# rdesc/autorally

Hardware: AMD Instinct MI355X
Metric: trajectory rollouts/s per MPPI solve (higher is better)
Workload: dtype f32

## Files before the change

autorally_amd/csrc/group_roles.hpp:

```cpp
#pragma once

#include "mppi_device.hpp"
#include "noise_device.hpp"

namespace mppi {

constexpr int kGRing = 16;
constexpr int kGCtlChunk = 4;

template <class SH>
struct GroupRoles {
  static constexpr int kPose = SH::NW, kCost = SH::NW + 1, kCtl = SH::NW + 2, kRng = SH::NW + 3;
  static constexpr int kWaves = SH::NW + 4;
  static_assert(kWaves <= (int)(sizeof(SH::fin) / sizeof(int)), "fin[]");
  static_assert(SH::kR == 16 || SH::kR == 8, "rollouts per group");
};
template <class SH>
__device__ __forceinline__ int group_j(int slot) { return slot & (SH::kR - 1); }
template <class SH>
__device__ __forceinline__ bool group_real(int slot) { return slot < SH::kR; }

template <class SH>
__device__ __forceinline__ int group_seq_min(SH &sh)
{
  int m = lds_peek(lds_addr(&sh.xseq[0][0]));
#pragma unroll
  for (int w = 1; w < SH::NW; w++) m = min(m, lds_peek(lds_addr(&sh.xseq[w][0])));
  return m;
}

struct MrgHalf {
  uint32_t s0, s1, s2;
};
__device__ __forceinline__ uint32_t fold_m(uint64_t x, uint32_t C, uint32_t m)
{
  x = (x >> 32) * C + (x & 0xffffffffULL);
  x = (x >> 32) * C + (x & 0xffffffffULL);
  x = (x >> 32) * C + (x & 0xffffffffULL);
  if (x >= m) x -= m;
  return (uint32_t)x;
}
template <class SH>
__device__ __forceinline__ MrgHalf group_rng_load(const RolloutArgs &a)
{
  const int lane = threadIdx.x & 63;
  const int j = group_j<SH>((lane >> 1) & 15), c = lane & 1;
  const int k = (int)blockIdx.x * SH::kR + j;
  const int K = a.K;
  MrgHalf g{0, 0, 0};
  if (a.inline_noise != 0 && lane < 2 * kRolloutsPerWave) {
    g.s0 = a.rng_in[(3 * c) * K + k]; g.s1 = a.rng_in[(3 * c + 1) * K + k]; g.s2 = a.rng_in[(3 * c + 2) * K + k];
  }
  return g;
}
template <class SH, bool PRE = false>
__device__ __forceinline__ void group_rng_wave(const RolloutArgs &a, SH &sh, const MrgHalf pre = MrgHalf{0, 0, 0})
{
  using R = GroupRoles<SH>;
  const int lane = threadIdx.x & 63;
  const int j = group_j<SH>((lane >> 1) & 15), c = lane & 1;
  const int k = (int)blockIdx.x * SH::kR + j;
  const int K = a.K, T = a.T;
  const bool active = lane < 2 * kRolloutsPerWave;
  const bool real = lane < 2 * SH::kR;
  int budget = spin_budget_init(a.spin_budget, T, a.fault_wave == R::kRng + 1);
  if (a.inline_noise != 0) {
    const uint32_t m = c ? (uint32_t)kM2 : (uint32_t)kM1, C = c ? kC2 : kC1;
    const uint32_t A = c ? (uint32_t)kA21 : (uint32_t)kA12, Bn = c ? (uint32_t)kA23N : (uint32_t)kA13N;
    MrgHalf g{0, 0, 0};
    if constexpr (PRE) {
      g = pre;
    } else if (active) {
      g.s0 = a.rng_in[(3 * c) * K + k]; g.s1 = a.rng_in[(3 * c + 1) * K + k]; g.s2 = a.rng_in[(3 * c + 2) * K + k];
    }
    const uint32_t a_ctl = lds_addr(&sh.ctl_pub[0]);
    const uint32_t a_mypub = lds_addr(&sh.rng_pub[lane]);
    int seen = 0;
    for (int t = 0; t < T; t++) {
      float2 e = make_float2(0.5f, 0.5f);
#ifdef MPPI_DIAG_NORNG
      e = make_float2(0.25f + 0.001f * (float)t, 0.5f);
#else
#pragma unroll
      for (int d = 0; d < 2; d++) {
        const uint32_t p = fold_m((uint64_t)A * (c ? g.s2 : g.s1) + (uint64_t)Bn * (m - g.s0), C, m);
        g.s0 = g.s1; g.s1 = g.s2; g.s2 = p;
        const uint32_t p2 = (uint32_t)__builtin_amdgcn_mov_dpp((int)p, 0xB1, 0xF, 0xF, false);
        uint32_t z = (p >= p2) ? p - p2 : p + (uint32_t)kM1 - p2;
        if (z == 0) z = (uint32_t)kM1;
        const float u = (float)z * 0x1p-32f;
        if (d == 0) e.x = u; else e.y = u;
      }
#endif
      const int need = t - kGRing + 1;
      while (seen < need && --budget > 0) {
        seen = lds_peek(a_ctl);
        if (seen < need) __builtin_amdgcn_s_sleep(2);
      }
      if (active && c == 0) *reinterpret_cast<float2 *>(&sh.eps[t & (kGRing - 1)][j][0]) = e;
      lds_publish(a_mypub, t + 1);
    }
    if (real) {
      a.rng_out[(3 * c) * K + k] = g.s0; a.rng_out[(3 * c + 1) * K + k] = g.s1; a.rng_out[(3 * c + 2) * K + k] = g.s2;
    }
  }
  spin_finish(budget, lds_addr(&sh.fail[0]), lds_addr(&sh.fin[R::kRng]));
}

template <class SH>
__device__ __forceinline__ void group_control_wave(const RolloutArgs &a, SH &sh, const uint32_t a_gate_open = 0)
{
  using R = GroupRoles<SH>;
  constexpr int NSW = SH::NSW;
  static_assert(kGCtlChunk == 4 && kGRing >= 2 * kGCtlChunk, "four steps per iteration, lanes 16 q + j");
  const int lane = threadIdx.x & 63;
  const int j = group_j<SH>(lane & 15), q = lane >> 4;
  const bool real = group_real<SH>(lane & 15);
  const int k = (int)blockIdx.x * SH::kR + j;
  const int K = a.K, T = a.T;
  const bool inl = a.inline_noise != 0;
  float2 *const noise = reinterpret_cast<float2 *>(a.noise);
  const float2 *const Useq = reinterpret_cast<const float2 *>(a.U);
  const bool noise_free_k = (k == 0);
  const bool pure_noise_k = (k >= a.k99);
  const uint32_t a_cd = lds_addr(&sh.cost_done[0]);
  const uint32_t a_mypub = lds_addr(&sh.ctl_pub[lane]);
  const uint32_t a_rng = lds_addr(&sh.rng_pub[0]);
  int budget = spin_budget_init(a.spin_budget, T, a.fault_wave == R::kCtl + 1);
  const bool gated = a_gate_open != 0;
  if (gated)
    while (lds_peek(a_gate_open) == 0 && --budget > 0) __builtin_amdgcn_s_sleep(1);
  int seen_x = 0, seen_c = 0, seen_r = 0;
  for (int t0 = 0, n = 1; t0 < T; t0 += n, n = kGCtlChunk) {
    const int t = t0 + q;
    const bool live = (t < T) & (q < n);
    const int tl = live ? t : T - 1;
    float2 Ut;
    if (gated) {
      const unsigned long long ub = __hip_atomic_load(reinterpret_cast<const unsigned long long *>(Useq + tl), __ATOMIC_RELAXED, __HIP_MEMORY_SCOPE_SYSTEM);
      Ut = make_float2(__uint_as_float((unsigned)ub), __uint_as_float((unsigned)(ub >> 32)));
    } else {
      Ut = Useq[tl];
    }
    float2 e = (live && !inl) ? noise[(size_t)tl * K + k] : make_float2(0.0f, 0.0f);
    const int tm = min(t0 + n, T) - 1;
    const int need_x = (tm >= kGRing) ? (tm - kGRing) * NSW + 1 : 0;
    const int need_c = tm - kGRing + 1;
    while ((seen_x < need_x || seen_c < need_c) && --budget > 0) {
      seen_x = group_seq_min(sh);
      seen_c = lds_peek(a_cd);
      if (seen_x < need_x || seen_c < need_c) __builtin_amdgcn_s_sleep(2);
    }
    if (inl) {
      while (seen_r < tm + 1 && --budget > 0) {
        seen_r = lds_peek(a_rng);
        if (seen_r < tm + 1) __builtin_amdgcn_s_sleep(1);
      }
#ifdef MPPI_DIAG_NOBM
      e = *reinterpret_cast<const float2 *>(&sh.eps[tl & (kGRing - 1)][j][0]);
#else
      e = box_muller(*reinterpret_cast<const float2 *>(&sh.eps[tl & (kGRing - 1)][j][0]));
#endif
    }
    if (live) {
      const bool nf = noise_free_k | (t < a.opt_delay);
      const float n0 = e.x * a.nu[0], n1 = e.y * a.nu[1];
      const float du0 = nf ? 0.0f : n0, du1 = nf ? 0.0f : n1;
      float u0 = nf ? Ut.x : (pure_noise_k ? n0 : Ut.x + n0);
      float u1 = nf ? Ut.y : (pure_noise_k ? n1 : Ut.y + n1);
      if (real) noise[(size_t)t * K + k] = make_float2(u0, u1);
      u0 = clampf(u0, a.u_lo[0], a.u_hi[0]);
      u1 = clampf(u1, a.u_lo[1], a.u_hi[1]);
      const int slot = t & (kGRing - 1);
      sh.ctl_b1[slot][j] = u0;
      sh.ctl_b1[slot][kRolloutsPerWave + j] = u1;
      *reinterpret_cast<float4 *>(&sh.ctl_rec[slot][j][0]) = make_float4(u0, u1, du0, du1);
    }
    lds_publish(a_mypub, tm + 1);
  }
  spin_finish(budget, lds_addr(&sh.fail[0]), lds_addr(&sh.fin[R::kCtl]));
}

template <class SH, bool AFFINE>
__device__ __forceinline__ void group_pose_wave(const RolloutArgs &a, SH &sh)
{
  using R = GroupRoles<SH>;
  constexpr int NSW = SH::NSW;
  static_assert(SH::kR == 16, "one step per iteration: 16-rollout groups only");
  const int lane = threadIdx.x & 63;
  const int j = lane & 15;
  const int T = a.T;
  const uint32_t a_seq0 = lds_addr(&sh.xseq[0][0]);
  const uint32_t a_cd = lds_addr(&sh.cost_done[0]);
  const uint32_t a_mypub = lds_addr(&sh.pose_pub[lane]);
  float x = a.state[0], y = a.state[1], yaw = a.state[2];
  int budget = spin_budget_init(a.spin_budget, T, a.fault_wave == R::kPose + 1), seen = 0, cdone = 0;
  float tf_p = 0.0f, tb_p = 0.0f;
  for (int t = 0; t <= T; t++) {
    float tf = 0.0f, tb = 0.0f;
    if (t < T) {
      const int need = t * NSW + 1;
      while (seen < need && --budget > 0) {
        seen = SH::kRecByAll ? group_seq_min(sh) : lds_peek(a_seq0);
        if (seen < need) __builtin_amdgcn_s_sleep(1);
      }
      const float4 r0 = *reinterpret_cast<const float4 *>(&sh.rec[t & (kGRing - 1)][j][0]);
      float spsi, cpsi;
#ifdef MPPI_DIAG_NOPOSE
      spsi = 0.0f; cpsi = 1.0f; tf = x; tb = y;
#else
      sincos_fast(yaw, spsi, cpsi);
      const float st[3] = {x, y, yaw};
      track_fetch<AFFINE>(a.cost, st, cpsi, spsi, tf, tb);
#endif
      const float sd0 = fmaf(cpsi, r0.y, -(spsi * r0.z));
      const float sd1 = fmaf(spsi, r0.y, cpsi * r0.z);
      const float sd2 = a.negate_yaw_der ? -r0.w : r0.w;
      x = fmaf(sd0, a.dt, x);
      y = fmaf(sd1, a.dt, y);
      yaw = fmaf(sd2, a.dt, yaw);
    }
    if (t > 0) {
      while (cdone < t - kGRing && --budget > 0) cdone = lds_peek(a_cd);
      if (lane < kRolloutsPerWave) *reinterpret_cast<float2 *>(&sh.tex[(t - 1) & (kGRing - 1)][lane][0]) = make_float2(tf_p, tb_p);
      lds_publish(a_mypub, t);
    }
    tf_p = tf; tb_p = tb;
  }
  spin_finish(budget, lds_addr(&sh.fail[0]), lds_addr(&sh.fin[R::kPose]));
}

template <int Q>
__device__ __forceinline__ float quad_bc(float v)
{
  return __int_as_float(__builtin_amdgcn_mov_dpp(__float_as_int(v), Q * 0x55, 0xF, 0xF, false));
}
__device__ __forceinline__ void quad_chain(float v, float d, float dt, int q, float &vq, float &v_out)
{
  const float v1 = fmaf(quad_bc<0>(d), dt, v);
  const float v2 = fmaf(quad_bc<1>(d), dt, v1);
  const float v3 = fmaf(quad_bc<2>(d), dt, v2);
  v_out = fmaf(quad_bc<3>(d), dt, v3);
  const float lo = (q == 0) ? v : v1, hi = (q == 2) ? v2 : v3;
  vq = (q < 2) ? lo : hi;
}
template <class SH, bool AFFINE>
__device__ __forceinline__ void group_pose_wave4(const RolloutArgs &a, SH &sh, const float x0, const float y0, const float yaw0,
                                                 const int budget_cut = 0);
template <class SH, bool AFFINE>
__device__ __forceinline__ void group_pose_wave4(const RolloutArgs &a, SH &sh)
{
  group_pose_wave4<SH, AFFINE>(a, sh, a.state[0], a.state[1], a.state[2]);
}
template <class SH, bool AFFINE>
__device__ __forceinline__ void group_pose_wave4(const RolloutArgs &a, SH &sh, const float x0, const float y0, const float yaw0,
                                                 const int budget_cut)
{
  using R = GroupRoles<SH>;
  constexpr int NSW = SH::NSW;
  static_assert(kRolloutsPerWave == 16 && kGRing >= 8, "lane = 4 j + q");
  const int lane = threadIdx.x & 63;
  const int j = group_j<SH>(lane >> 2), q = lane & 3;
  const int T = a.T;
  const uint32_t a_seq0 = lds_addr(&sh.xseq[0][0]);
  const uint32_t a_cd = lds_addr(&sh.cost_done[0]);
  const uint32_t a_mypub = lds_addr(&sh.pose_pub[lane]);
  float x = x0, y = y0, yaw = yaw0;
  int budget = spin_budget_init(a.spin_budget, T, a.fault_wave == R::kPose + 1 || budget_cut != 0), seen = 0, cdone = 0;
  for (int t0 = 0; t0 < T; t0 += 4) {
    const int t = t0 + q;
    const int tend = min(t0 + 4, T);
    const int need = (tend - 1) * NSW + 1;
    while (seen < need && --budget > 0) {
      seen = SH::kRecByAll ? group_seq_min(sh) : lds_peek(a_seq0);
      if (seen < need) __builtin_amdgcn_s_sleep(1);
    }
    const float4 r0 = *reinterpret_cast<const float4 *>(&sh.rec[t & (kGRing - 1)][j][0]);
    float yaw_q, yaw_n, x_q, x_n, y_q, y_n;
    quad_chain(yaw, a.negate_yaw_der ? -r0.w : r0.w, a.dt, q, yaw_q, yaw_n);
    float spsi, cpsi, tf = 0.0f, tb = 0.0f;
#ifdef MPPI_DIAG_NOPOSE
    spsi = 0.0f; cpsi = 1.0f;
#else
    sincos_fast(yaw_q, spsi, cpsi);
#endif
    quad_chain(x, fmaf(cpsi, r0.y, -(spsi * r0.z)), a.dt, q, x_q, x_n);
    quad_chain(y, fmaf(spsi, r0.y, cpsi * r0.z), a.dt, q, y_q, y_n);
#ifdef MPPI_DIAG_NOPOSE
    tf = x_q; tb = y_q;
#else
    const float st[3] = {x_q, y_q, yaw_q};
    track_fetch<AFFINE>(a.cost, st, cpsi, spsi, tf, tb);
#endif
    x = x_n; y = y_n; yaw = yaw_n;
    while (cdone < tend - kGRing && --budget > 0) cdone = lds_peek(a_cd);
    if (t < T) *reinterpret_cast<float2 *>(&sh.tex[t & (kGRing - 1)][j][0]) = make_float2(tf, tb);
    lds_publish(a_mypub, tend);
  }
  spin_finish(budget, lds_addr(&sh.fail[0]), lds_addr(&sh.fin[R::kPose]));
}

template <class SH>
__device__ __forceinline__ float group_settle(SH &sh, int budget, float J)
{
  using R = GroupRoles<SH>;
  const int lane = threadIdx.x & 63;
  const uint32_t a_fin = lds_addr(&sh.fin[(lane < R::kWaves) ? lane : 0]);
  for (;;) {
    const int v = (lane == R::kCost) ? 1 : lds_peek_lanes(a_fin);
    const bool all = __builtin_amdgcn_ballot_w64(v != 0) == ~0ull;
    if (all || --budget <= 0) break;
    __builtin_amdgcn_s_sleep(1);
  }
  if (budget <= 0 || lds_peek(lds_addr(&sh.fail[0])) != 0) J = __builtin_nanf("");
  return J;
}

template <class SH, bool CTRL>
__device__ __forceinline__ void group_cost_wave(const RolloutArgs &a, SH &sh)
{
  using R = GroupRoles<SH>;
  const int lane = threadIdx.x & 63;
  static_assert(SH::kR == 16, "one step per iteration: 16-rollout groups only");
  const int j = lane & 15;
  const int k = (int)blockIdx.x * kRolloutsPerWave + j;
  const int T = a.T;
  const uint32_t a_mydone = lds_addr(&sh.cost_done[lane]);
  const uint32_t a_pose = lds_addr(&sh.pose_pub[0]);
  int crash = 0, budget = spin_budget_init(a.spin_budget, T, a.fault_wave == R::kCost + 1), seen = 0;
  float J = 0.0f;
  for (int t = 0; t < T; t++) {
    const double rt = a.inv_t[t];
    while (seen < t + 1 && --budget > 0) {
      seen = lds_peek(a_pose);
      if (seen < t + 1) __builtin_amdgcn_s_sleep(1);
    }
    const float4 r0 = *reinterpret_cast<const float4 *>(&sh.rec[t & (kGRing - 1)][j][0]);
    const float4 r1 = *reinterpret_cast<const float4 *>(&sh.ctl_rec[t & (kGRing - 1)][j][0]);
    const float2 tx = *reinterpret_cast<const float2 *>(&sh.tex[t & (kGRing - 1)][j][0]);
    lds_publish(a_mydone, t + 1);
    const int rc = (int)((t > 0) & (fabsf(r0.x) >= kRollCrash));
#ifdef MPPI_DIAG_NOCOST
    crash |= rc;
    int crash_new = crash;
    const float Jn = J + r0.y + r1.x + tx.x + (float)rt;
#else
    CostTerms ct;
    cost_terms_a<CTRL>(a.cost, a.nu, r0.y, r0.z, r1.x, r1.y, r1.z, r1.w, ct);
    crash |= rc;
    int crash_new = crash;
    const float c = cost_terms_b(a.cost, ct, tx.x, tx.y, crash_new);
    const float Jn = running_mean(J, c, t, rt);
#endif
    J = (t > 0) ? Jn : J;
    crash = (t > 0) ? crash_new : crash;
  }
  J = group_settle(sh, budget, J);
  a.costs[k] = J + 0.0f;
}

template <int Q>
__device__ __forceinline__ int quad_bc_i(int v)
{
  return __builtin_amdgcn_mov_dpp(v, Q * 0x55, 0xF, 0xF, false);
}
template <class SH, bool CTRL>
__device__ __forceinline__ void group_cost_wave4(const RolloutArgs &a, SH &sh)
{
  using R = GroupRoles<SH>;
  const int lane = threadIdx.x & 63;
  const int j = group_j<SH>(lane >> 2), q = lane & 3;
  const int k = (int)blockIdx.x * SH::kR + j;
  const int T = a.T;
  const uint32_t a_mydone = lds_addr(&sh.cost_done[lane]);
  const uint32_t a_pose = lds_addr(&sh.pose_pub[0]);
  int crash = 0, budget = spin_budget_init(a.spin_budget, T, a.fault_wave == R::kCost + 1), seen = 0;
  float J = 0.0f;
  for (int t0 = 0; t0 < T; t0 += 4) {
    const int t = t0 + q;
    const int tend = min(t0 + 4, T);
    while (seen < tend && --budget > 0) {
      seen = lds_peek(a_pose);
      if (seen < tend) __builtin_amdgcn_s_sleep(1);
    }
    const float4 r0 = *reinterpret_cast<const float4 *>(&sh.rec[t & (kGRing - 1)][j][0]);
    const float4 r1 = *reinterpret_cast<const float4 *>(&sh.ctl_rec[t & (kGRing - 1)][j][0]);
    const float2 tx = *reinterpret_cast<const float2 *>(&sh.tex[t & (kGRing - 1)][j][0]);
    lds_publish(a_mydone, tend);
    const bool counted = (t > 0) & (t < T);
    int e = (int)(fabsf(r0.x) >= kRollCrash) | (int)(tx.x >= a.cost.boundary_threshold) | (int)(tx.y >= a.cost.boundary_threshold);
    e = counted ? e : 0;
    const int c0 = crash | quad_bc_i<0>(e), c1 = c0 | quad_bc_i<1>(e), c2 = c1 | quad_bc_i<2>(e), c3 = c2 | quad_bc_i<3>(e);
    const int lo = (q == 0) ? c0 : c1, hi = (q == 2) ? c2 : c3;
    int crash_q = (q < 2) ? lo : hi;
    crash = c3;
#ifdef MPPI_DIAG_NOCOST
    const float c = r0.y + r1.x + tx.x + (float)crash_q;
#else
    CostTerms ct;
    cost_terms_a<CTRL>(a.cost, a.nu, r0.y, r0.z, r1.x, r1.y, r1.z, r1.w, ct);
    const float c = cost_terms_b(a.cost, ct, tx.x, tx.y, crash_q);
#endif
#pragma unroll
    for (int l = 0; l < 4; l++) {
      const int tl = t0 + l;
      const float cl = (l == 0) ? quad_bc<0>(c) : (l == 1) ? quad_bc<1>(c) : (l == 2) ? quad_bc<2>(c) : quad_bc<3>(c);
      if (tl > 0 && tl < T) {
#ifdef MPPI_DIAG_NOCOST
        J = J + cl + (float)a.inv_t[tl];
#else
        J = running_mean(J, cl, tl, a.inv_t[tl]);
#endif
      }
    }
  }
  J = group_settle(sh, budget, J);
  if (q == 0 && group_real<SH>(lane >> 2)) a.costs[k] = J + 0.0f;
}

}
```

autorally_amd/csrc/rollout_m44.hip:

```cpp
#include "group_roles.hpp"
#include "mppi_kernels.hpp"

namespace mppi {

typedef float m44_f4 __attribute__((ext_vector_type(4)));
constexpr int kM44H = 64;

struct M44Shared {
  static constexpr int NW = 4;
  static constexpr int NSW = 1;
  static constexpr int kR = 16;
  static constexpr bool kRecByAll = true;
  int xseq[NW][64];
  float rec[kGRing][kRolloutsPerWave][4];
  int cost_done[64];
  float ctl_b1[kGRing][64];
  float ctl_rec[kGRing][kRolloutsPerWave][4];
  int ctl_pub[64];
  float tex[kGRing][kRolloutsPerWave][2];
  int pose_pub[64];
  float eps[kGRing][kRolloutsPerWave][2];
  int rng_pub[64];
  int fail[4];
  int fin[8];
  float gstate[8];
  int gate_open[8];
  m44_f4 wo[4][64];
  float dump[NW][64 * kGRing];
};

template <int NHID>
constexpr int m44_q_bias() { return 2; }
template <int NHID>
constexpr int m44_q_hidden() { return 2 + (NHID + 3) / 4; }
template <int NHID>
constexpr int m44_q_out() { return m44_q_hidden<NHID>() + (NHID - 1) * 16; }
template <int NHID>
constexpr int m44_q_total() { return m44_q_out<NHID>() + 5; }

template <int Q>
__device__ __forceinline__ float m44_qp(float v)
{
  return __int_as_float(__builtin_amdgcn_mov_dpp(__float_as_int(v), Q, 0xF, 0xF, false));
}
__device__ __forceinline__ void m44_transpose(const float (&in)[4], float (&out)[4], bool hi, bool od)
{
  float t[4];
  {
    const float x0 = m44_qp<0x4E>(hi ? in[0] : in[2]);
    const float x1 = m44_qp<0x4E>(hi ? in[1] : in[3]);
    t[0] = hi ? x0 : in[0];
    t[2] = hi ? in[2] : x0;
    t[1] = hi ? x1 : in[1];
    t[3] = hi ? in[3] : x1;
  }
  {
    const float y0 = m44_qp<0xB1>(od ? t[0] : t[1]);
    const float y1 = m44_qp<0xB1>(od ? t[2] : t[3]);
    out[0] = od ? y0 : t[0];
    out[1] = od ? t[1] : y0;
    out[2] = od ? y1 : t[2];
    out[3] = od ? t[3] : y1;
  }
}

template <int K>
__device__ __forceinline__ void m44_step(m44_f4 &d, const float (&T)[4], const float *w)
{
  d = __builtin_amdgcn_mfma_f32_4x4x1f32(T[K & 3], w[K], d, 4, K >> 2, 0);
}
template <int K0>
__device__ __forceinline__ void m44_steps16(m44_f4 &d, const float (&T)[4], const float *w)
{
#define S4(K) m44_step<K>(d, T, w); m44_step<K + 1>(d, T, w); m44_step<K + 2>(d, T, w); m44_step<K + 3>(d, T, w);
  S4(K0) S4(K0 + 4) S4(K0 + 8) S4(K0 + 12)
#undef S4
}
__device__ __forceinline__ void m44_tanh(const m44_f4 &d, float bs, float (&act)[4])
{
  const f32x2 a01 = tanh_bias2(f32x2{d[0], d[1]}, f32x2{bs, bs});
  const f32x2 a23 = tanh_bias2(f32x2{d[2], d[3]}, f32x2{bs, bs});
  act[0] = a01.x; act[1] = a01.y; act[2] = a23.x; act[3] = a23.y;
}

template <int CTRL>
__device__ __forceinline__ float m44_dpp_add(float acc, float src)
{
  return acc + __int_as_float(__builtin_amdgcn_update_dpp(0, __float_as_int(src), CTRL, 0xF, 0xF, true));
}
__device__ __forceinline__ float m44_out_tree(const f32x2 (&q)[4], const f32x2 (&p)[4], const float (&T)[4])
{
  f32x2 Q = q[0] * f32x2{T[0], T[0]}, P = p[0] * f32x2{T[0], T[0]};
#pragma unroll
  for (int s = 1; s < 4; s++) {
    Q = __builtin_elementwise_fma(q[s], f32x2{T[s], T[s]}, Q);
    P = __builtin_elementwise_fma(p[s], f32x2{T[s], T[s]}, P);
  }
  {
    auto x = __builtin_amdgcn_permlane32_swap(__float_as_uint(Q.x), __float_as_uint(P.x), false, false);
// ... 231 lines not shown
```

autorally_amd/csrc/rollout_oct.hip:

```cpp
#include "mfma_net.hpp"
#include "group_roles.hpp"
#include "mppi_kernels.hpp"

namespace mppi {

template <int H, int NHID>
struct OctShared {
  static constexpr int NW = 4;
  static constexpr int NSW = NHID;
  static constexpr int kR = 16;
  static constexpr bool kRecByAll = false;
  float xb[2][NW][64][4];
  int xseq[NW][64];
  float rec[kGRing][kRolloutsPerWave][4];
  int cost_done[64];
  float ctl_b1[kGRing][64];
  float ctl_rec[kGRing][kRolloutsPerWave][4];
  int ctl_pub[64];
  float tex[kGRing][kRolloutsPerWave][2];
  int pose_pub[64];
  float eps[kGRing][kRolloutsPerWave][2];
  int rng_pub[64];
  int fail[4];
  int fin[8];
};

__device__ __forceinline__ void oct_poll(const uint32_t (&a_seq)[3], const uint32_t (&a_x)[3], int &f, f32x4 (&oth)[3])
{
  int f0, f1, f2;
  asm volatile(
      "ds_read_b32 %0, %6\n\tds_read_b128 %3, %9\n\t"
      "ds_read_b32 %1, %7\n\tds_read_b128 %4, %10\n\t"
      "ds_read_b32 %2, %8\n\tds_read_b128 %5, %11\n\t"
      "s_waitcnt lgkmcnt(0)"
      : "=&v"(f0), "=&v"(f1), "=&v"(f2), "=&v"(oth[0]), "=&v"(oth[1]), "=&v"(oth[2])
      : "v"(a_seq[0]), "v"(a_seq[1]), "v"(a_seq[2]), "v"(a_x[0]), "v"(a_x[1]), "v"(a_x[2])
      : "memory");
  f = __builtin_amdgcn_readfirstlane(min(min(f0, f1), f2));
}

template <int H, int NHID, int W>
__device__ __forceinline__ void oct_dynamics(const RolloutArgs &a, OctShared<H, NHID> &sh)
{
  using N = MfmaNet<H, NHID>;
  constexpr int MT = N::MT, KSH = N::KSH, NSW = NHID;
  static_assert(MT == 4, "one M tile per dynamics wave: 64-wide hidden layers");
  const int lane = threadIdx.x & 63;
  const int j = lane & 15, g = lane >> 4;
  const int T = a.T;

  float A0[2], B0[4], AH[(NHID - 1) * KSH + 1], Bh[(NHID - 1) * 4 + 1], AL[KSH], BL[4];
  A0[0] = a.wpack[(W * 2 + 0) * 64 + lane];
  A0[1] = a.wpack[(W * 2 + 1) * 64 + lane];
#pragma unroll
  for (int r = 0; r < 4; r++) B0[r] = a.wpack[(N::nA + W * 4 + r) * 64 + lane] * kTanhScale;
#pragma unroll
  for (int l = 1; l < NHID; l++) {
#pragma unroll
    for (int s = 0; s < KSH; s++)
      AH[(l - 1) * KSH + s] = a.wpack[(N::nA0 + (l - 1) * N::nAH + W * KSH + s) * 64 + lane];
#pragma unroll
    for (int r = 0; r < 4; r++) Bh[(l - 1) * 4 + r] = a.wpack[(N::nA + l * MT * 4 + W * 4 + r) * 64 + lane] * kTanhScale;
  }
#pragma unroll
  for (int s = 0; s < KSH; s++) AL[s] = a.wpack[(N::nA0 + (NHID - 1) * N::nAH + s) * 64 + lane];
#pragma unroll
  for (int r = 0; r < 4; r++) BL[r] = a.wpack[(N::nA + NHID * MT * 4 + r) * 64 + lane];

  const uint32_t a_myseq = lds_addr(&sh.xseq[W][lane]);
  const uint32_t a_xmine = lds_addr(&sh.xb[0][W][lane][0]);
  uint32_t a_seq[3], a_xo[3];
#pragma unroll
  for (int i = 0; i < 3; i++) {
    a_seq[i] = lds_addr(&sh.xseq[(W + 1 + i) & 3][0]);
    a_xo[i] = lds_addr(&sh.xb[0][(W + 1 + i) & 3][lane][0]);
  }
  const uint32_t a_pub = lds_addr(&sh.ctl_pub[0]);
  const uint32_t a_cd = lds_addr(&sh.cost_done[0]);
  constexpr uint32_t kXbParity = 4 * 64 * 4 * 4;

  typedef const volatile int __attribute__((address_space(3))) *lds_int_p;
  typedef const volatile float __attribute__((address_space(3))) *lds_float_p;
  const lds_int_p p_pub = (lds_int_p)&sh.ctl_pub[0];
  const lds_int_p p_cd = (lds_int_p)&sh.cost_done[0];
  const lds_float_p p_b1 = (lds_float_p)&sh.ctl_b1[0][lane];

  float s3 = a.state[3], s4 = a.state[4], s5 = a.state[5], s6 = a.state[6];
  int budget = spin_budget_init(a.spin_budget, T, a.fault_wave == W + 1);
  while (lds_peek(a_pub) < 1 && --budget > 0) __builtin_amdgcn_s_sleep(1);
  float b1_next = sh.ctl_b1[0][lane];
  asm volatile("" : "+v"(b1_next));
  int cp_v = 0, cd_v = 0;
  float b1n_v = 0.0f;

// ... 140 lines not shown
```

autorally_amd/csrc/rollout_row.hip:

```cpp
#include "group_roles.hpp"
#include "mppi_kernels.hpp"

namespace mppi {

#ifdef MPPI_ROW_STAMPS
__device__ unsigned long long g_row_stamps[16];
#define RSTAMP(i)                                                                                         \
  do {                                                                                                    \
    if (blockIdx.x == 0 && (threadIdx.x & 63) == 0) {                                                     \
      unsigned long long t__;                                                                             \
      asm volatile("s_memtime %0\n\ts_waitcnt lgkmcnt(0)" : "=s"(t__)::"memory");                           \
      g_row_stamps[i] = t__;                                                                              \
    }                                                                                                     \
  } while (0)
#else
#define RSTAMP(i) do { } while (0)
#endif

template <int H>
struct RowShared {
  static constexpr int NW = 4;
  static constexpr int NSW = 1;
  static constexpr bool kRecByAll = true;
  static constexpr int kR = 16;
  int xseq[NW][64];
  float rec[kGRing][kRolloutsPerWave][4];
  int cost_done[64];
  float ctl_b1[kGRing][64];
  float ctl_rec[kGRing][kRolloutsPerWave][4];
  int ctl_pub[64];
  float tex[kGRing][kRolloutsPerWave][2];
  int pose_pub[64];
  float eps[kGRing][kRolloutsPerWave][2];
  int rng_pub[64];
  int fail[4];
  int fin[8];
  float gstate[8];
  int gate_open[8];
  float dump[NW][64 * 2 + (kGRing - 1) * kRolloutsPerWave * 4];
};

template <int H, bool TREE>
struct RowWeights {
  f32x2 w1[kNetIn], w2[H], w3[TREE ? 4 : H];
  f32x2 b1s, b2s, b3;
};

constexpr int kRowPackEntries = 40;
template <int H, bool TREE>
__device__ __forceinline__ void row_load(const float *rowpack, int p, RowWeights<H, TREE> &W)
{
  static_assert(H == 32, "entry layout of pack_row_weights");
  const float4 *pk = reinterpret_cast<const float4 *>(rowpack) + p;
#pragma unroll
  for (int i = 0; i < 3; i++) {
    const float4 v = pk[i * 16];
    W.w1[2 * i] = f32x2{v.x, v.y};
    W.w1[2 * i + 1] = f32x2{v.z, v.w};
  }
#pragma unroll
  for (int i = 0; i < H / 2; i++) {
    const float4 v = pk[(3 + i) * 16];
    W.w2[2 * i] = f32x2{v.x, v.y};
    W.w2[2 * i + 1] = f32x2{v.z, v.w};
    if constexpr (!TREE) {
      const float4 u = pk[(3 + H / 2 + i) * 16];
      W.w3[2 * i] = f32x2{u.x, u.y};
      W.w3[2 * i + 1] = f32x2{u.z, u.w};
    }
  }
  const float4 b = pk[35 * 16];
  W.b1s = f32x2{b.x, b.y};
  W.b2s = f32x2{b.z, b.w};
  if constexpr (TREE) {
    const float4 u = pk[37 * 16], v = pk[38 * 16], c = pk[39 * 16];
    W.w3[0] = f32x2{u.x, u.y};
    W.w3[1] = f32x2{u.z, u.w};
    W.w3[2] = f32x2{v.x, v.y};
    W.w3[3] = f32x2{v.z, v.w};
    W.b3 = f32x2{c.x, c.y};
  } else {
    const float4 c = pk[36 * 16];
    W.b3 = f32x2{c.x, c.y};
  }
}

template <int Q>
__device__ __forceinline__ float row_bc(float a)
{
  return __int_as_float(__builtin_amdgcn_mov_dpp(__float_as_int(a), 0x150 + Q, 0xF, 0xF, false));
}
template <int Q>
__device__ __forceinline__ f32x2 row_bc2(f32x2 a)
{
  return __builtin_bit_cast(f32x2, (long long)__builtin_amdgcn_mov_dpp(__builtin_bit_cast(long long, a), 0x150 + Q, 0xF, 0xF, false));
}
template <int Q>
__device__ __forceinline__ void row_dot_step(f32x2 &z, f32x2 &b, const f32x2 *w, f32x2 a)
{
  z = __builtin_elementwise_fma(w[2 * Q], f32x2{b.x, b.x}, z);
  __builtin_amdgcn_sched_barrier(0);
  const f32x2 bn = row_bc2<(Q + 1 < 16 ? Q + 1 : 15)>(a);
  __builtin_amdgcn_sched_barrier(0);
  z = __builtin_elementwise_fma(w[2 * Q + 1], f32x2{b.y, b.y}, z);
  __builtin_amdgcn_sched_barrier(0);
  b = bn;
}
__device__ __forceinline__ f32x2 row_dot_bc(const f32x2 *w, f32x2 a)
{
  f32x2 z = {0.0f, 0.0f};
  f32x2 b = row_bc2<0>(a);
  __builtin_amdgcn_sched_barrier(0);
#define RD4(Q) row_dot_step<Q>(z, b, w, a); row_dot_step<Q + 1>(z, b, w, a); row_dot_step<Q + 2>(z, b, w, a); row_dot_step<Q + 3>(z, b, w, a);
  RD4(0) RD4(4) RD4(8) RD4(12)
#undef RD4
  return z;
}

template <int CTRL>
__device__ __forceinline__ float dpp_add(float acc, float src)
{
  return acc + __int_as_float(__builtin_amdgcn_update_dpp(0, __float_as_int(src), CTRL, 0xF, 0xF, true));
}
__device__ __forceinline__ float row_out_tree(const f32x2 *w3, f32x2 a)
{
  const f32x2 ax = {a.x, a.x}, ay = {a.y, a.y};
  const f32x2 v01 = __builtin_elementwise_fma(w3[1], ay, w3[0] * ax);
  const f32x2 v23 = __builtin_elementwise_fma(w3[3], ay, w3[2] * ax);
  float v0 = dpp_add<0x128>(v01.x, v23.x);
  const float v1 = dpp_add<0x128>(v01.y, v23.y);
  v0 = dpp_add<0x141>(v0, v1);
  v0 = dpp_add<0xB1>(v0, v0);
  v0 = dpp_add<0x4E>(v0, v0);
  return v0;
}

template <int H, bool TREE, int Q>
__device__ __forceinline__ void row_step(const RolloutArgs &a, const RowWeights<H, TREE> &W, f32x2 &sp, f32x2 &un, const int t0,
                                         const uint32_t a_rec, const uint32_t a_myseq, const volatile int __attribute__((address_space(3))) *p_pub,
                                         const volatile f32x2 __attribute__((address_space(3))) *&pu,
                                         const volatile f32x2 __attribute__((address_space(3))) *p_u0, int &cp, int &budget)
{
  constexpr int kSlotF2 = kRolloutsPerWave * 2;
  constexpr uint32_t kRecStride = sizeof(float) * kRolloutsPerWave * 4;
  const int t = t0 + Q;
  const f32x2 u = un;
  const f32x2 slo = TREE ? f32x2{row_bc<0>(sp.x), row_bc<4>(sp.x)} : f32x2{row_bc<0>(sp.x), row_bc<0>(sp.y)};
  const f32x2 shi = TREE ? f32x2{row_bc<8>(sp.x), row_bc<12>(sp.x)} : f32x2{row_bc<1>(sp.x), row_bc<1>(sp.y)};
  if constexpr (TREE) asm volatile("ds_write_b32 %0, %1 offset:%2" ::"v"(a_rec), "v"(sp.x), "n"(Q * kRecStride) : "memory");
  else asm volatile("ds_write_b64 %0, %1 offset:%2" ::"v"(a_rec), "v"(sp), "n"(Q * kRecStride) : "memory");
  if constexpr (Q == 3) lds_publish(a_myseq, t + 1);
  f32x2 z = {0.0f, 0.0f};
  z = __builtin_elementwise_fma(W.w1[0], f32x2{slo.x, slo.x}, z);
  z = __builtin_elementwise_fma(W.w1[1], f32x2{slo.y, slo.y}, z);
  z = __builtin_elementwise_fma(W.w1[2], f32x2{shi.x, shi.x}, z);
  z = __builtin_elementwise_fma(W.w1[3], f32x2{shi.y, shi.y}, z);
  z = __builtin_elementwise_fma(W.w1[4], f32x2{u.x, u.x}, z);
  z = __builtin_elementwise_fma(W.w1[5], f32x2{u.y, u.y}, z);
  int cp_v = 0;
  if constexpr (Q == 0) cp_v = *p_pub;
  if constexpr (Q == 3) pu = p_u0 + ((t + 1) & (kGRing - 1)) * kSlotF2;
  constexpr int kUn = (Q == 3) ? 0 : (Q + 1) * kSlotF2;
  un = pu[kUn];
  const f32x2 a0 = tanh_bias2(z, W.b1s);
  const f32x2 a1 = tanh_bias2(row_dot_bc(W.w2, a0), W.b2s);
  const int want = t + 2;
  if constexpr (Q == 0) cp = __builtin_amdgcn_readfirstlane(cp_v);
  asm volatile("" : "+v"(un));
  if constexpr (TREE) {
    const float d = row_out_tree(W.w3, a1) + W.b3.x;
    sp.x = fmaf(d, a.dt, sp.x);
    asm volatile("" : "+v"(sp.x));
  } else {
    const f32x2 d = row_dot_bc(W.w3, a1) + W.b3;
    sp = __builtin_elementwise_fma(d, f32x2{a.dt, a.dt}, sp);
    asm volatile("" : "+v"(sp));
  }
  if (__builtin_expect(cp < want, 0)) {
    while (cp < want && --budget > 0) {
      cp = __builtin_amdgcn_readfirstlane(*p_pub);
      un = pu[kUn];
    }
    asm volatile("" : "+v"(un));
  }
}

template <int H, bool TREE, bool GATED = false>
__device__ __forceinline__ void row_dynamics(const RolloutArgs &a, RowShared<H> &sh, const int w)
{
  static_assert(H == 32, "row_dot_bc: 32 activations, two per lane of a 16-lane row");
  static_assert(kGRing % 4 == 0, "aligned chunks of four steps inside the ring");
  const int lane = threadIdx.x & 63;
  const int r = lane >> 4, p = lane & 15;
  const int jr = 4 * w + r;
  const bool odd = (p & 1) != 0;
  const int T = a.T;
  RowWeights<H, TREE> W;
  row_load<H, TREE>(a.wpack, p, W);
#pragma unroll
  for (int k = 0; k < H; k++) asm volatile("" : "+v"(W.w2[k]));
#pragma unroll
  for (int k = 0; k < (TREE ? 4 : H); k++) asm volatile("" : "+v"(W.w3[k]));

  const uint32_t a_myseq = lds_addr(&sh.xseq[w][lane]);
  typedef const volatile int __attribute__((address_space(3))) *lds_int_p;
  typedef const volatile f32x2 __attribute__((address_space(3))) *lds_f2_p;
  const lds_int_p p_pub = (lds_int_p)&sh.ctl_pub[0];
  uint32_t a_u0 = lds_addr(&sh.ctl_rec[0][jr][0]);
  asm volatile("" : "+v"(a_u0));
  const lds_f2_p p_u = (lds_f2_p)a_u0;
  const uint32_t a_rec0 = TREE ? (((p & 3) == 0) ? lds_addr(&sh.rec[0][jr][p >> 2]) : lds_addr(&sh.dump[w][2 * lane]))
                               : ((p < 2) ? lds_addr(&sh.rec[0][jr][2 * p]) : lds_addr(&sh.dump[w][2 * lane]));
  constexpr uint32_t kRecStride = sizeof(float) * kRolloutsPerWave * 4;

  int budget = spin_budget_init(a.spin_budget, T, a.fault_wave == w + 1);
  f32x2 sp;
  if constexpr (GATED) {
    const uint32_t a_go = lds_addr(&sh.gate_open[0]);
    while (lds_peek(a_go) == 0 && --budget > 0) __builtin_amdgcn_s_sleep(1);
    const volatile float *gs = sh.gstate;
    sp = TREE ? f32x2{gs[3 + (p >> 2)], 0.0f} : odd ? f32x2{gs[5], gs[6]} : f32x2{gs[3], gs[4]};
  } else {
    sp = TREE ? f32x2{a.state[3 + (p >> 2)], 0.0f} : odd ? f32x2{a.state[5], a.state[6]} : f32x2{a.state[3], a.state[4]};
  }
  if (w == 0) RSTAMP(2);
  int cp = 0;
  while ((cp = __builtin_amdgcn_readfirstlane(*p_pub)) < 1 && --budget > 0) __builtin_amdgcn_s_sleep(1);
  if (w == 0) RSTAMP(3);
  lds_f2_p pu = p_u;
  f32x2 un = pu[0];
  asm volatile("" : "+v"(un));

  const int NS = T - 1;
  for (int t0 = 0; t0 < NS; t0 += 4) {
    const uint32_t a_rec = a_rec0 + (uint32_t)(t0 & (kGRing - 1)) * kRecStride;
    row_step<H, TREE, 0>(a, W, sp, un, t0, a_rec, a_myseq, p_pub, pu, p_u, cp, budget);
    if (t0 + 1 >= NS) break;
    row_step<H, TREE, 1>(a, W, sp, un, t0, a_rec, a_myseq, p_pub, pu, p_u, cp, budget);
    if (t0 + 2 >= NS) break;
    row_step<H, TREE, 2>(a, W, sp, un, t0, a_rec, a_myseq, p_pub, pu, p_u, cp, budget);
    if (t0 + 3 >= NS) break;
    row_step<H, TREE, 3>(a, W, sp, un, t0, a_rec, a_myseq, p_pub, pu, p_u, cp, budget);
  }
  if (w == 0) RSTAMP(4);
  {
    const int t = T - 1;
    if constexpr (TREE) asm volatile("ds_write_b32 %0, %1" ::"v"(a_rec0 + (uint32_t)(t & (kGRing - 1)) * kRecStride), "v"(sp.x) : "memory");
    else asm volatile("ds_write_b64 %0, %1" ::"v"(a_rec0 + (uint32_t)(t & (kGRing - 1)) * kRecStride), "v"(sp) : "memory");
    lds_publish(a_myseq, t + 1);
  }
  spin_finish(budget, lds_addr(&sh.fail[0]), lds_addr(&sh.fin[w]));
}

template <int H, bool AFFINE, bool CTRL, bool TREE, bool GATED = false>
__device__ __forceinline__ void row_group(const RolloutArgs &a, RowShared<H> &sh)
{
  using SH = RowShared<H>;
  using R = GroupRoles<SH>;
  const int lane = threadIdx.x & 63;
  const int role = __builtin_amdgcn_readfirstlane(threadIdx.x >> 6);
  if (role == 0) RSTAMP(0);
  MrgHalf g0{0, 0, 0};
  if (role == R::kRng) g0 = group_rng_load<SH>(a);
  if (role == 0) {
#pragma unroll
    for (int w = 0; w < 4; w++) sh.xseq[w][lane] = 0;
    sh.cost_done[lane] = 0;
    sh.ctl_pub[lane] = 0;
    sh.pose_pub[lane] = 0;
    sh.rng_pub[lane] = 0;
    sh.fail[lane & 3] = 0;
    sh.fin[lane & 7] = 0;
    sh.gate_open[lane & 7] = 0;
  }
  __syncthreads();
  if (role == 0) RSTAMP(1);
#ifdef MPPI_ROW_RIDER_PRIO
  if (role >= 4) __builtin_amdgcn_s_setprio(MPPI_ROW_RIDER_PRIO);
#endif
  if (role < 4) row_dynamics<H, TREE, GATED>(a, sh, role);
  else if (role == R::kCost) { group_cost_wave4<SH, CTRL>(a, sh); RSTAMP(5); }
  else if (role == R::kCtl) { group_control_wave(a, sh, GATED ? lds_addr(&sh.gate_open[0]) : 0u); RSTAMP(6); }
  else if (role == R::kPose) {
    if constexpr (GATED) {
      const int shut = group_gate_wait(a, sh);
      const volatile float *gs = sh.gstate;
      const float x0 = gs[0], y0 = gs[1], yaw0 = gs[2];
      group_pose_wave4<SH, AFFINE>(a, sh, x0, y0, yaw0, shut);
    } else {
      group_pose_wave4<SH, AFFINE>(a, sh);
    }
    RSTAMP(7);
  }
  else { group_rng_wave<SH, true>(a, sh, g0); RSTAMP(8); }
}

template <int H, bool AFFINE, bool CTRL, bool TREE>
__global__ __launch_bounds__(512) void rollout_row_kernel(const RolloutArgs a)
{
  __shared__ __attribute__((aligned(16))) RowShared<H> sh;
  row_group<H, AFFINE, CTRL, TREE>(a, sh);
}
template <int H, bool AFFINE, bool CTRL, bool TREE>
__global__ __launch_bounds__(512) void rollout_row_gated_kernel(const RolloutArgs a)
{
  __shared__ __attribute__((aligned(16))) RowShared<H> sh;
  row_group<H, AFFINE, CTRL, TREE, true>(a, sh);
}

template <int H, bool AFFINE, bool CTRL, bool TREE, int NB>
__global__ __launch_bounds__(512) void rollout_row_batch_kernel(const QuadBatchArgsT<NB> b)
{
  __shared__ __attribute__((aligned(16))) RowShared<H> sh;
#define MPPI_ROW_BODY(A)                                                                                   \
  do {                                                                                                     \
    if ((int)blockIdx.x >= (A).K / kRolloutsPerWave) return;      \
    row_group<H, AFFINE, CTRL, TREE>((A), sh);                                                             \
  } while (0)
  MPPI_BATCH_DISPATCH(NB, b, MPPI_ROW_BODY);
#undef MPPI_ROW_BODY
}

template <int H, bool AFFINE, bool CTRL, bool TREE, int NB>
__global__ __launch_bounds__(512) void rollout_row_batch_gated_kernel(const QuadBatchArgsT<NB> b)
{
// ... 88 lines not shown
```

autorally_amd/csrc/rollout_row64.hip:

```cpp
#include "group_roles.hpp"
#include "mppi_kernels.hpp"

namespace mppi {

constexpr int kH64 = 64;
constexpr int kPF = 8;

template <int NHID, int R>
struct Row64Shared {
  static constexpr int NW = R / 2;
  static constexpr int NSW = 1;
  static constexpr int kR = R;
  static constexpr bool kRecByAll = true;
  f32x2 wl[NHID - 1][kH64][32];
  int xseq[NW][64];
  float rec[kGRing][kRolloutsPerWave][4];
  int cost_done[64];
  float ctl_b1[kGRing][64];
  float ctl_rec[kGRing][kRolloutsPerWave][4];
  int ctl_pub[64];
  float tex[kGRing][kRolloutsPerWave][2];
  int pose_pub[64];
  float eps[kGRing][kRolloutsPerWave][2];
  int rng_pub[64];
  int fail[4];
  int fin[16];
  float dump[NW][64 * kGRing];
};

template <int NHID>
struct Row64Regs {
  f32x2 w1[kNetIn];
  f32x2 bs[NHID];
  f32x2 q[2], p[2];
  float bo;
};
template <int NHID>
constexpr int row64_reg_entries() { return 3 + (NHID + 1) / 2 + 3; }

template <int NHID>
__device__ __forceinline__ void row64_load(const float *pack, int g, Row64Regs<NHID> &W)
{
  constexpr int NB = (NHID + 1) / 2;
  const float4 *pk = reinterpret_cast<const float4 *>(pack) + g;
#pragma unroll
  for (int i = 0; i < 3; i++) {
    const float4 v = pk[i * 32];
    W.w1[2 * i] = f32x2{v.x, v.y};
    W.w1[2 * i + 1] = f32x2{v.z, v.w};
  }
#pragma unroll
  for (int i = 0; i < NB; i++) {
    const float4 v = pk[(3 + i) * 32];
    W.bs[2 * i] = f32x2{v.x, v.y};
    if (2 * i + 1 < NHID) W.bs[2 * i + 1] = f32x2{v.z, v.w};
  }
  const float4 u = pk[(3 + NB) * 32], v = pk[(4 + NB) * 32], c = pk[(5 + NB) * 32];
  W.q[0] = f32x2{u.x, u.y};
  W.q[1] = f32x2{u.z, u.w};
  W.p[0] = f32x2{v.x, v.y};
  W.p[1] = f32x2{v.z, v.w};
  W.bo = c.x;
}

template <int Q>
__device__ __forceinline__ float r64_bc(float a)
{
  return __int_as_float(__builtin_amdgcn_mov_dpp(__float_as_int(a), 0x150 + Q, 0xF, 0xF, false));
}
__device__ __forceinline__ void r64_rows(float a, float &lo, float &up)
{
  auto x = __builtin_amdgcn_permlane16_swap(__float_as_uint(a), __float_as_uint(a), false, false);
  lo = __uint_as_float(x[0]);
  up = __uint_as_float(x[1]);
}
template <int P>
__device__ __forceinline__ f32x2 r64_pair(f32x2 L, f32x2 U)
{
  const f32x2 src = (P < 16) ? L : U;
  return __builtin_bit_cast(f32x2, (long long)__builtin_amdgcn_mov_dpp(__builtin_bit_cast(long long, src), 0x150 + (P & 15), 0xF, 0xF, false));
}
typedef const volatile f32x2 __attribute__((address_space(3))) *r64_lds_p;
template <int P>
__device__ __forceinline__ void r64_step(f32x2 &z, f32x2 &b, f32x2 *ring, r64_lds_p base, f32x2 L, f32x2 U)
{
  constexpr int K = 2 * P;
  const f32x2 w0 = ring[K % kPF];
  if constexpr (K + kPF < kH64) ring[K % kPF] = base[(K + kPF) * 32];
  z = __builtin_elementwise_fma(w0, f32x2{b.x, b.x}, z);
  __builtin_amdgcn_sched_barrier(0);
  const f32x2 bn = r64_pair<(P + 1 < kH64 / 2 ? P + 1 : kH64 / 2 - 1)>(L, U);
  const f32x2 w1 = ring[(K + 1) % kPF];
  if constexpr (K + 1 + kPF < kH64) ring[(K + 1) % kPF] = base[(K + 1 + kPF) * 32];
  __builtin_amdgcn_sched_barrier(0);
  z = __builtin_elementwise_fma(w1, f32x2{b.y, b.y}, z);
  __builtin_amdgcn_sched_barrier(0);
  b = bn;
}
template <int P0>
__device__ __forceinline__ void r64_steps16(f32x2 &z, f32x2 &b, f32x2 *ring, r64_lds_p base, f32x2 L, f32x2 U)
{
// ... 202 lines not shown
```

Measured before the change: 106.2 million.

## Use double-precision MRG reduction, drop unused ctl_b1 LDS, shorten last-step dependency chains

The MRG32k3a step in the RNG wave now uses a double-precision fma, floor and modulo reduction in place of the triple 64-bit fold. The ctl_b1 LDS buffer and its writes are removed for layouts that never read it (row, row64, m44), which cuts LDS footprint and store traffic. The final step of the row dynamics is peeled so it publishes its sequence counter early. The pose and cost waves now wait only on that earlier counter for the last chunk, and the cost wave computes control cost terms before waiting on pose, so the tail of the pipeline overlaps more. The new code adds wait-condition logic that must stay consistent across the wave roles.

```diff
diff --git a/autorally_amd/csrc/group_roles.hpp b/autorally_amd/csrc/group_roles.hpp
--- a/autorally_amd/csrc/group_roles.hpp
+++ b/autorally_amd/csrc/group_roles.hpp
@@ -32,14 +32,6 @@
 struct MrgHalf {
   uint32_t s0, s1, s2;
 };
-__device__ __forceinline__ uint32_t fold_m(uint64_t x, uint32_t C, uint32_t m)
-{
-  x = (x >> 32) * C + (x & 0xffffffffULL);
-  x = (x >> 32) * C + (x & 0xffffffffULL);
-  x = (x >> 32) * C + (x & 0xffffffffULL);
-  if (x >= m) x -= m;
-  return (uint32_t)x;
-}
 template <class SH>
 __device__ __forceinline__ MrgHalf group_rng_load(const RolloutArgs &a)
 {
@@ -65,7 +57,6 @@
   const bool real = lane < 2 * SH::kR;
   int budget = spin_budget_init(a.spin_budget, T, a.fault_wave == R::kRng + 1);
   if (a.inline_noise != 0) {
-    const uint32_t m = c ? (uint32_t)kM2 : (uint32_t)kM1, C = c ? kC2 : kC1;
     const uint32_t A = c ? (uint32_t)kA21 : (uint32_t)kA12, Bn = c ? (uint32_t)kA23N : (uint32_t)kA13N;
     MrgHalf g{0, 0, 0};
     if constexpr (PRE) {
@@ -73,6 +64,9 @@
     } else if (active) {
       g.s0 = a.rng_in[(3 * c) * K + k]; g.s1 = a.rng_in[(3 * c + 1) * K + k]; g.s2 = a.rng_in[(3 * c + 2) * K + k];
     }
+    const double md = c ? (double)kM2 : (double)kM1, inv_m = c ? 1.0 / (double)kM2 : 1.0 / (double)kM1;
+    const double Ad = (double)A, nBn = -(double)Bn;
+    double d0 = (double)g.s0, d1 = (double)g.s1, d2 = (double)g.s2;
     const uint32_t a_ctl = lds_addr(&sh.ctl_pub[0]);
     const uint32_t a_mypub = lds_addr(&sh.rng_pub[lane]);
     int seen = 0;
@@ -83,8 +77,13 @@
 #else
 #pragma unroll
       for (int d = 0; d < 2; d++) {
-        const uint32_t p = fold_m((uint64_t)A * (c ? g.s2 : g.s1) + (uint64_t)Bn * (m - g.s0), C, m);
-        g.s0 = g.s1; g.s1 = g.s2; g.s2 = p;
+        const double pd = __builtin_fma(nBn, d0, Ad * (c ? d2 : d1));
+        const double kq = __builtin_floor(pd * inv_m);
+        double r = __builtin_fma(-kq, md, pd);
+        r = (r < 0.0) ? r + md : r;
+        r = (r >= md) ? r - md : r;
+        d0 = d1; d1 = d2; d2 = r;
+        const uint32_t p = (uint32_t)r;
         const uint32_t p2 = (uint32_t)__builtin_amdgcn_mov_dpp((int)p, 0xB1, 0xF, 0xF, false);
         uint32_t z = (p >= p2) ? p - p2 : p + (uint32_t)kM1 - p2;
         if (z == 0) z = (uint32_t)kM1;
@@ -101,7 +100,7 @@
       lds_publish(a_mypub, t + 1);
     }
     if (real) {
-      a.rng_out[(3 * c) * K + k] = g.s0; a.rng_out[(3 * c + 1) * K + k] = g.s1; a.rng_out[(3 * c + 2) * K + k] = g.s2;
+      a.rng_out[(3 * c) * K + k] = (uint32_t)d0; a.rng_out[(3 * c + 1) * K + k] = (uint32_t)d1; a.rng_out[(3 * c + 2) * K + k] = (uint32_t)d2;
     }
   }
   spin_finish(budget, lds_addr(&sh.fail[0]), lds_addr(&sh.fin[R::kRng]));
@@ -172,8 +171,10 @@
       u0 = clampf(u0, a.u_lo[0], a.u_hi[0]);
       u1 = clampf(u1, a.u_lo[1], a.u_hi[1]);
       const int slot = t & (kGRing - 1);
-      sh.ctl_b1[slot][j] = u0;
-      sh.ctl_b1[slot][kRolloutsPerWave + j] = u1;
+      if constexpr (SH::kCtlB1) {
+        sh.ctl_b1[slot][j] = u0;
+        sh.ctl_b1[slot][kRolloutsPerWave + j] = u1;
+      }
       *reinterpret_cast<float4 *>(&sh.ctl_rec[slot][j][0]) = make_float4(u0, u1, du0, du1);
     }
     lds_publish(a_mypub, tm + 1);
@@ -270,7 +271,7 @@
   for (int t0 = 0; t0 < T; t0 += 4) {
     const int t = t0 + q;
     const int tend = min(t0 + 4, T);
-    const int need = (tend - 1) * NSW + 1;
+    const int need = ((tend < T ? tend : T - 1) - 1) * NSW + 1;
     while (seen < need && --budget > 0) {
       seen = SH::kRecByAll ? group_seq_min(sh) : lds_peek(a_seq0);
       if (seen < need) __builtin_amdgcn_s_sleep(1);
@@ -374,17 +375,40 @@
   const int T = a.T;
   const uint32_t a_mydone = lds_addr(&sh.cost_done[lane]);
   const uint32_t a_pose = lds_addr(&sh.pose_pub[0]);
-  int crash = 0, budget = spin_budget_init(a.spin_budget, T, a.fault_wave == R::kCost + 1), seen = 0;
+  const uint32_t a_seq0 = lds_addr(&sh.xseq[0][0]);
+  int crash = 0, budget = spin_budget_init(a.spin_budget, T, a.fault_wave == R::kCost + 1), seen = 0, seen_x = 0;
   float J = 0.0f;
   for (int t0 = 0; t0 < T; t0 += 4) {
     const int t = t0 + q;
     const int tend = min(t0 + 4, T);
-    while (seen < tend && --budget > 0) {
-      seen = lds_peek(a_pose);
-      if (seen < tend) __builtin_amdgcn_s_sleep(1);
+    const bool last = tend == T;
+    if (last) {
+      const int need_r = (T - 1) * SH::NSW + 1;
+      while (seen_x < need_r && --budget > 0) {
+        seen_x = SH::kRecByAll ? group_seq_min(sh) : lds_peek(a_seq0);
+        if (seen_x < need_r) __builtin_amdgcn_s_sleep(1);
+      }
+    } else {
+      while (seen < tend && --budget > 0) {
+        seen = lds_peek(a_pose);
+        if (seen < tend) __builtin_amdgcn_s_sleep(1);
+      }
     }
     const float4 r0 = *reinterpret_cast<const float4 *>(&sh.rec[t & (kGRing - 1)][j][0]);
     const float4 r1 = *reinterpret_cast<const float4 *>(&sh.ctl_rec[t & (kGRing - 1)][j][0]);
+#ifndef MPPI_DIAG_NOCOST
+    CostTerms ct;
+    cost_terms_a<CTRL>(a.cost, a.nu, r0.y, r0.z, r1.x, r1.y, r1.z, r1.w, ct);
+#endif
+    if (last) {
+#ifndef MPPI_DIAG_NOCOST
+      asm volatile("" : "+v"(ct.control_cost), "+v"(ct.speed_cost), "+v"(ct.stabilizing_cost));
+#endif
+      while (seen < tend && --budget > 0) {
+        seen = lds_peek(a_pose);
+        if (seen < tend) __builtin_amdgcn_s_sleep(1);
+      }
+    }
     const float2 tx = *reinterpret_cast<const float2 *>(&sh.tex[t & (kGRing - 1)][j][0]);
     lds_publish(a_mydone, tend);
     const bool counted = (t > 0) & (t < T);
@@ -397,8 +421,6 @@
 #ifdef MPPI_DIAG_NOCOST
     const float c = r0.y + r1.x + tx.x + (float)crash_q;
 #else
-    CostTerms ct;
-    cost_terms_a<CTRL>(a.cost, a.nu, r0.y, r0.z, r1.x, r1.y, r1.z, r1.w, ct);
     const float c = cost_terms_b(a.cost, ct, tx.x, tx.y, crash_q);
 #endif
 #pragma unroll
diff --git a/autorally_amd/csrc/rollout_m44.hip b/autorally_amd/csrc/rollout_m44.hip
--- a/autorally_amd/csrc/rollout_m44.hip
+++ b/autorally_amd/csrc/rollout_m44.hip
@@ -11,10 +11,10 @@
   static constexpr int NSW = 1;
   static constexpr int kR = 16;
   static constexpr bool kRecByAll = true;
+  static constexpr bool kCtlB1 = false;
   int xseq[NW][64];
   float rec[kGRing][kRolloutsPerWave][4];
   int cost_done[64];
-  float ctl_b1[kGRing][64];
   float ctl_rec[kGRing][kRolloutsPerWave][4];
   int ctl_pub[64];
   float tex[kGRing][kRolloutsPerWave][2];
diff --git a/autorally_amd/csrc/rollout_oct.hip b/autorally_amd/csrc/rollout_oct.hip
--- a/autorally_amd/csrc/rollout_oct.hip
+++ b/autorally_amd/csrc/rollout_oct.hip
@@ -10,6 +10,7 @@
   static constexpr int NSW = NHID;
   static constexpr int kR = 16;
   static constexpr bool kRecByAll = false;
+  static constexpr bool kCtlB1 = true;
   float xb[2][NW][64][4];
   int xseq[NW][64];
   float rec[kGRing][kRolloutsPerWave][4];
diff --git a/autorally_amd/csrc/rollout_row.hip b/autorally_amd/csrc/rollout_row.hip
--- a/autorally_amd/csrc/rollout_row.hip
+++ b/autorally_amd/csrc/rollout_row.hip
@@ -23,10 +23,10 @@
   static constexpr int NSW = 1;
   static constexpr bool kRecByAll = true;
   static constexpr int kR = 16;
+  static constexpr bool kCtlB1 = false;
   int xseq[NW][64];
   float rec[kGRing][kRolloutsPerWave][4];
   int cost_done[64];
-  float ctl_b1[kGRing][64];
   float ctl_rec[kGRing][kRolloutsPerWave][4];
   int ctl_pub[64];
   float tex[kGRing][kRolloutsPerWave][2];
@@ -135,7 +135,7 @@
   return v0;
 }
 
-template <int H, bool TREE, int Q>
+template <int H, bool TREE, int Q, bool LAST = false>
 __device__ __forceinline__ void row_step(const RolloutArgs &a, const RowWeights<H, TREE> &W, f32x2 &sp, f32x2 &un, const int t0,
                                          const uint32_t a_rec, const uint32_t a_myseq, const volatile int __attribute__((address_space(3))) *p_pub,
                                          const volatile f32x2 __attribute__((address_space(3))) *&pu,
@@ -149,7 +149,7 @@
   const f32x2 shi = TREE ? f32x2{row_bc<8>(sp.x), row_bc<12>(sp.x)} : f32x2{row_bc<1>(sp.x), row_bc<1>(sp.y)};
   if constexpr (TREE) asm volatile("ds_write_b32 %0, %1 offset:%2" ::"v"(a_rec), "v"(sp.x), "n"(Q * kRecStride) : "memory");
   else asm volatile("ds_write_b64 %0, %1 offset:%2" ::"v"(a_rec), "v"(sp), "n"(Q * kRecStride) : "memory");
-  if constexpr (Q == 3) lds_publish(a_myseq, t + 1);
+  if constexpr (Q == 3 || LAST) lds_publish(a_myseq, t + 1);
   f32x2 z = {0.0f, 0.0f};
   z = __builtin_elementwise_fma(W.w1[0], f32x2{slo.x, slo.x}, z);
   z = __builtin_elementwise_fma(W.w1[1], f32x2{slo.y, slo.y}, z);
@@ -231,16 +231,26 @@
   f32x2 un = pu[0];
   asm volatile("" : "+v"(un));
 
-  const int NS = T - 1;
-  for (int t0 = 0; t0 < NS; t0 += 4) {
+  const int NS = T - 1, NL = NS - 1;
+  for (int t0 = 0; t0 < NL; t0 += 4) {
     const uint32_t a_rec = a_rec0 + (uint32_t)(t0 & (kGRing - 1)) * kRecStride;
     row_step<H, TREE, 0>(a, W, sp, un, t0, a_rec, a_myseq, p_pub, pu, p_u, cp, budget);
-    if (t0 + 1 >= NS) break;
+    if (t0 + 1 >= NL) break;
     row_step<H, TREE, 1>(a, W, sp, un, t0, a_rec, a_myseq, p_pub, pu, p_u, cp, budget);
-    if (t0 + 2 >= NS) break;
+    if (t0 + 2 >= NL) break;
     row_step<H, TREE, 2>(a, W, sp, un, t0, a_rec, a_myseq, p_pub, pu, p_u, cp, budget);
-    if (t0 + 3 >= NS) break;
+    if (t0 + 3 >= NL) break;
     row_step<H, TREE, 3>(a, W, sp, un, t0, a_rec, a_myseq, p_pub, pu, p_u, cp, budget);
+  }
+  if (NL >= 0) {
+    const int t0 = NL & ~3;
+    const uint32_t a_rec = a_rec0 + (uint32_t)(t0 & (kGRing - 1)) * kRecStride;
+    switch (NL & 3) {
+      case 0: row_step<H, TREE, 0, true>(a, W, sp, un, t0, a_rec, a_myseq, p_pub, pu, p_u, cp, budget); break;
+      case 1: row_step<H, TREE, 1, true>(a, W, sp, un, t0, a_rec, a_myseq, p_pub, pu, p_u, cp, budget); break;
+      case 2: row_step<H, TREE, 2, true>(a, W, sp, un, t0, a_rec, a_myseq, p_pub, pu, p_u, cp, budget); break;
+      default: row_step<H, TREE, 3, true>(a, W, sp, un, t0, a_rec, a_myseq, p_pub, pu, p_u, cp, budget); break;
+    }
   }
   if (w == 0) RSTAMP(4);
   {
diff --git a/autorally_amd/csrc/rollout_row64.hip b/autorally_amd/csrc/rollout_row64.hip
--- a/autorally_amd/csrc/rollout_row64.hip
+++ b/autorally_amd/csrc/rollout_row64.hip
@@ -12,11 +12,11 @@
   static constexpr int NSW = 1;
   static constexpr int kR = R;
   static constexpr bool kRecByAll = true;
+  static constexpr bool kCtlB1 = false;
   f32x2 wl[NHID - 1][kH64][32];
   int xseq[NW][64];
   float rec[kGRing][kRolloutsPerWave][4];
   int cost_done[64];
-  float ctl_b1[kGRing][64];
   float ctl_rec[kGRing][kRolloutsPerWave][4];
   int ctl_pub[64];
   float tex[kGRing][kRolloutsPerWave][2];
```

New measurement: 105.6 million. About the same (-0.6%).
